# honglianghe/CDNet

Measured on AMD Instinct MI355X. Metric: tiles/sec (train fwd+bwd+Adam), 256x256, higher is better.
Workload: dtype fp32

## Files before the change

cdnet_amd/_lib.py:

```python
import ctypes as C
import os

_HERE = os.path.dirname(os.path.abspath(__file__))
LIB_PATH = os.environ.get('CDNET_LIB_PATH') or os.path.join(_HERE, 'libcdnet_hip.so')

_vp, _i, _sz, _f = C.c_void_p, C.c_int, C.c_size_t, C.c_float

class WgradReduceDesc(C.Structure):
    _fields_ = [('slab', C.c_void_p), ('dw', C.c_void_p)] + [(n, C.c_int) for n in (
        'ksplit', 'npar', 'ci_blocks', 'co_blocks', 'taps', 'CI', 'CO', 'Csrc_real', 'Cin_real', 'src_coff', 'Cout', 'mode', 'block0', 'blocks')]


SIGNATURES = {
    'cdnet_abi_version': (_i, []),
    'cdnet_abi_sizeof': (_sz, [C.c_char_p]),
    'cdnet_last_error': (C.c_char_p, []),
    'cdnet_build_info': (C.c_char_p, []),
    'cdnet_spin': (_i, [_i, _vp]),
    'cdnet_box_copy': (_i, [_vp, _vp, _sz, _vp]),
    'cdnet_box_mfma': (_i, [_vp, _vp, _vp, _i, _i, _i, _vp]),
    'cdnet_ddm_codes': (_i, [_vp, _i, _i, _i, _i, _vp, _i, _i, _vp, _vp, _vp]),
    'cdnet_ddm_normalize': (_i, [_vp, _vp, _i, _i, _i, _vp, _vp]),
    'cdnet_probmaps': (_i, [_vp, _vp, _i, _i, _i, _i, _vp, _vp, _vp]),
    'cdnet_tta_boost_argmax': (_i, [_vp, _vp, _vp, _vp, _i, _i, _vp, _i, _i, _vp, _vp, _vp, _vp, _vp, _vp]),
    'cdnet_fuse_sum': (_i, [_vp, _i, _i, _i, _i, _i, _i, _vp, _i, _i, _vp]),
    'cdnet_upsample_bilinear_backward': (_i, [_vp, _i, _i, _i, _i, _i, _i, _i, _i, _vp, _vp]),
    'cdnet_s2d_to_nhwc': (_i, [_vp, _i, _i, _i, _i, _vp, _vp]),
    'cdnet_fuse_sum_f32': (_i, [_vp, _i, _i, _i, _i, _i, _i, _vp, _i, _i, _vp]),
    'cdnet_upsample_bilinear_backward_f32': (_i, [_vp, _i, _i, _i, _i, _i, _i, _i, _i, _vp, _vp]),
    'cdnet_s2d_to_nhwc_f32': (_i, [_vp, _i, _i, _i, _i, _vp, _vp]),
    'cdnet_bn_backward_stats': (_i, [_vp, _vp, _vp, _vp, _vp, _sz, _vp, _vp]),
    'cdnet_bn_backward_apply': (_i, [_vp, _vp, _vp, _vp]),
    'cdnet_bn_backward_finalize': (_i, [_vp, _vp, _vp, _vp, _vp, _i, _vp, _vp]),
    'cdnet_conv_ws_eligible': (_i, [_vp]),
    'cdnet_grad_sum': (_i, [_vp, _i, _vp, C.c_longlong, _i, _vp, _vp]),
    'cdnet_grad_sum_f32': (_i, [_vp, _i, _vp, C.c_longlong, _i, _vp, _vp]),
    'cdnet_label_pair_histogram': (_i, [_vp, _vp, _i, _i, _i, _i, _vp, _vp, _vp, _vp, _vp, _vp]),
    'cdnet_remap_label': (_i, [_vp, _i, _i, _i, _vp, _vp, _vp, _vp]),
    'cdnet_watershed_workspace_bytes': (_sz, [_i, _i, _i]),
    'cdnet_watershed_process': (_i, [_vp, _i, _i, _i, _i, _vp, _sz, _vp, _vp, _vp, _vp]),
    'cdnet_fill_label_process': (_i, [_vp, _i, _i, _i, _i, _vp, _sz, _vp, _vp]),
    'cdnet_tile_postproc_workspace_bytes': (_sz, [_i, _i, _i, _i]),
    'cdnet_tile_postproc': (_i, [_vp, _vp, _vp, _i, _i, _i, _i, _vp, _i, _i, _i, _i, _vp, _sz] + [_vp] * 10),
    'cdnet_cc_workspace_bytes': (_sz, [_i, _i, _i]),
    'cdnet_cc_chain': (_i, [_vp, _i, _i, _i, _i, _i, _i, _vp, _sz, _vp, _vp, _vp, _vp, _vp, _vp]),
    'cdnet_mask_views_argmax': (_i, [_vp, _i, _i, _i, _vp, _i, _i, _vp, _vp, _vp]),
    'cdnet_tile_mask_postproc_workspace_bytes': (_sz, [_i, _i, _i, _i]),
    'cdnet_tile_mask_postproc': (_i, [_vp, _i, _i, _i, _i, _i, _i, _vp, _sz] + [_vp] * 8),
    'cdnet_dilate_labels': (_i, [_vp, _i, _i, _i, _i, _vp, _vp]),
    'cdnet_conv_packed_weight_elems': (_sz, [_i] * 6),
    'cdnet_pack_conv_weights': (_i, [_vp, _vp] + [_i] * 7 + [_vp]),
    'cdnet_pack_conv_weights_scaled': (_i, [_vp, _vp, _vp] + [_i] * 7 + [_vp]),
    'cdnet_pack_batch_table_bytes': (_sz, [_i]),
    'cdnet_pack_conv_weights_batch': (_i, [_vp, _i, _vp, _sz, _i, _vp]),
    'cdnet_conv_forward': (_i, [_vp, _vp]),
    'cdnet_src_materialize': (_i, [_vp, _i, _i, _i, _vp, _vp]),
    'cdnet_input_pack': (_i, [_vp, _i, _i, _i, _i, _vp, _vp]),
    'cdnet_input_pack_f32': (_i, [_vp, _i, _i, _i, _i, _vp, _vp]),
    'cdnet_bn_fold_eval': (_i, [_vp, _vp, _vp, _vp, _vp, _f, _i, _vp, _vp, _vp]),
    'cdnet_bn_finalize_train': (_i, [_vp, _i, _i, _f, _vp, _vp, _vp, _f, _f, _vp, _vp, _vp, _vp, _vp, _vp, _vp]),
    'cdnet_dam_head_forward': (_i, [_vp, _vp, _vp, _vp, _i, _i, _i, _vp, _vp, _vp, _vp]),
    'cdnet_final_conv1x1': (_i, [_vp, _vp, _vp, _i, _i, _i, _i, _vp, _vp]),
    'cdnet_bias_grad_workspace_floats': (_sz, [_i]),
    'cdnet_bias_grad': (_i, [_vp, _sz, _i, _vp, _sz, _vp, _vp]),
    'cdnet_bias_grad_f32': (_i, [_vp, _sz, _i, _vp, _sz, _vp, _vp]),
    'cdnet_final_conv1x1_backward_workspace_floats': (_sz, []),
    'cdnet_final_conv1x1_backward': (_i, [_vp, _vp, _vp, _i, _i, _i, _i, _vp, _vp, _sz, _vp, _vp, _vp]),
# ... 102 lines not shown
```

cdnet_amd/csrc/conv32.hip:

```cpp
#include <type_traits>
#include "common.h"
#include "conv_args.h"
#include "launch.h"
#include <stdlib.h>

using namespace cdnet;

typedef __attribute__((ext_vector_type(8))) __bf16 bf16x8;
typedef __attribute__((ext_vector_type(2))) __bf16 bf16x2;
typedef __attribute__((ext_vector_type(16))) float f32x16;
typedef __attribute__((ext_vector_type(2))) float f32x2;
typedef unsigned u32x4 __attribute__((ext_vector_type(4)));
typedef float f32x4 __attribute__((ext_vector_type(4)));

namespace {

__device__ __forceinline__ void split8(const float *v, u32x4 &hi, u32x4 &lo) {
#pragma unroll
    for (int k = 0; k < 4; ++k) {
        const f32x2 x = {v[2 * k], v[2 * k + 1]};
        const bf16x2 h = __builtin_convertvector(x, bf16x2);
        const unsigned hb = __builtin_bit_cast(unsigned, h);
        const f32x2 hf = {__builtin_bit_cast(float, hb << 16), __builtin_bit_cast(float, hb & 0xffff0000u)};
        const bf16x2 l = __builtin_convertvector(x - hf, bf16x2);
        hi[k] = hb;
        lo[k] = __builtin_bit_cast(unsigned, l);
    }
}

constexpr int CK = 16;
constexpr int PSTR = CK * 2 + 16;
constexpr int XF_MAX = 2048;

template <int TH, int TW, int BN, int TAPS>
struct Lds32 {
    static constexpr int NPIX = (TH + 2) * (TW + 2);
    static constexpr int A_PLANE = NPIX * PSTR;
    static constexpr int B_PLANE = TAPS * CK * BN * 2;
    static constexpr int STAGE = 2 * A_PLANE + 2 * B_PLANE;
    static constexpr int STATS_BYTES = 4 * 2 * BN * 4;
    static constexpr int MAIN = ((STAGE > STATS_BYTES ? STAGE : STATS_BYTES) + 15) / 16 * 16;
    static int bytes(int ctot) { return MAIN + 2 * ((ctot + 7) / 8 * 8) * 4; }
};


template <int MPW, int NPW, int TW>
__device__ __forceinline__ void store_tile_f32(const ConvArgs &A, const f32x16 (&acc)[MPW][NPW], int n, int y0, int x0, int mblock0, int nblock0,
                                               int half, int l31, int cout0, int pa_, int pb_) {
    const int Ho = A.H * A.ostride, Wo = A.W * A.ostride;
    float *out = reinterpret_cast<float *>(A.out);
    const float *eres = reinterpret_cast<const float *>(A.eres);
    const bool full = y0 + 16 <= A.H && x0 + TW <= A.W && cout0 + (nblock0 + NPW) * 32 <= A.Cout && A.ostride == 1 && TW == 16 &&
                      !(A.debug & 16);
    if (full) {
        const int cs = A.out_cstride, ce = A.Cout;
        float *tb = out + (((size_t)n * A.H + y0) * A.W + x0) * cs + A.out_coff;
        const float *te = eres ? eres + (((size_t)n * A.H + y0) * A.W + x0) * ce : nullptr;
#pragma unroll
        for (int ni = 0; ni < NPW; ++ni) {
            const int co = cout0 + (nblock0 + ni) * 32 + l31;
            const float osc = A.oscale ? A.oscale[co] : 1.f;
            const float osh = fmaf(A.bias ? A.bias[co] : 0.f, osc, A.oshift ? A.oshift[co] : 0.f);
            const float esc = (eres && A.eres_scale) ? A.eres_scale[co] : 1.f;
            const float esh = (eres && A.eres_shift) ? A.eres_shift[co] : 0.f;
            float *ob = tb + co;
#pragma unroll
            for (int mi = 0; mi < MPW; ++mi) {
                const int rowb = ((mblock0 + mi) * 2) * A.W + 4 * half;
                float ev[16];
                if (eres) {
#pragma unroll
                    for (int r = 0; r < 16; ++r) {
                        const int p = (r & 3) + 8 * (r >> 2);
                        ev[r] = te[(rowb + (p / 16) * A.W + (p % 16)) * ce + co];
                    }
                }
#pragma unroll
                for (int r = 0; r < 16; ++r) {
                    const int p = (r & 3) + 8 * (r >> 2);
                    const int off = (rowb + (p / 16) * A.W + (p % 16)) * cs;
                    float v = fmaf(acc[mi][ni][r], osc, osh);
                    if (A.orelu) v = fmaxf(v, 0.f);
                    if (eres) {
                        v = fmaf(ev[r], esc, esh) + v;
                        if (A.eres_relu) v = fmaxf(v, 0.f);
                    }
// ... 12 lines not shown
        const float esc = (A.eres && A.eres_scale && cok) ? A.eres_scale[co] : 1.f;
        const float esh = (A.eres && A.eres_shift && cok) ? A.eres_shift[co] : 0.f;
#pragma unroll
        for (int mi = 0; mi < MPW; ++mi) {
            float ev[16];
            if (A.eres) {
#pragma unroll
                for (int r = 0; r < 16; ++r) {
                    const int m = (mblock0 + mi) * 32 + (r & 3) + 8 * (r >> 2) + 4 * half;
                    int y = y0 + m / TW, x = x0 + m % TW;
                    y = y < A.H ? y : A.H - 1; x = x < A.W ? x : A.W - 1;
                    ev[r] = eres[(((size_t)n * A.H + y) * A.W + x) * A.Cout + (cok ? co : 0)];
                }
            }
#pragma unroll
            for (int r = 0; r < 16; ++r) {
                const int m = (mblock0 + mi) * 32 + (r & 3) + 8 * (r >> 2) + 4 * half;
                const int y = y0 + m / TW, x = x0 + m % TW;
                float v = fmaf(acc[mi][ni][r], osc, osh);
                if (A.orelu) v = fmaxf(v, 0.f);
                if (A.eres) {
                    v = fmaf(ev[r], esc, esh) + v;
                    if (A.eres_relu) v = fmaxf(v, 0.f);
                }
                if (cok && y < A.H && x < A.W) {
                    const size_t opix = ((size_t)n * Ho + (y * A.ostride + pa_)) * Wo + (x * A.ostride + pb_);
                    out[opix * A.out_cstride + A.out_coff + co] = v;
                }
            }
        }
    }
}

template <int TH, int TW, int BN, int WM, int WN, int TAPS>
__global__ __launch_bounds__(256, 2) void conv_f32_kernel(ConvArgs A) {
    using L = Lds32<TH, TW, BN, TAPS>;
    constexpr int HW_ = TW + 2, NPIX = L::NPIX;
    constexpr int MT = TH * TW / 32, NT = BN / 32;
    constexpr int MPW = MT / WM, NPW = NT / WN;
    constexpr int VPP = CK / 8;
    constexpr int NA = (NPIX * VPP + 255) / 256;
    constexpr int NBV = 2 * L::B_PLANE / 16;
    constexpr int NB = (NBV + 255) / 256;
    static_assert(MT % WM == 0 && NT % WN == 0 && WM * WN == 4, "wave tiling");

    extern __shared__ __attribute__((aligned(16))) unsigned char smem[];
    unsigned char *lds_a = smem;
    unsigned char *lds_b = smem + 2 * L::A_PLANE;
    float (*s_stats)[2][BN] = reinterpret_cast<float (*)[2][BN]>(smem);
    float *s_xf = reinterpret_cast<float *>(smem + L::MAIN);

    const int tid = threadIdx.x, lane = tid & 63, wave = tid >> 6;
    const int wm = wave / WN, wn = wave % WN;
    const int half = lane >> 5, l31 = lane & 31;
    const int c0n = A.src[0].C, ctot = c0n + (A.nsrc > 1 ? A.src[1].C : 0);
    const int xfs = (ctot + 7) / 8 * 8;
    for (int c = tid; c < ctot; c += 256) {
        const ConvSrc &S = c < c0n ? A.src[0] : A.src[1];
        const int cc = c < c0n ? c : c - c0n;
        s_xf[c] = S.scale ? S.scale[cc] : 1.f;
        s_xf[xfs + c] = S.shift ? S.shift[cc] : 0.f;
    }

    const int tiles_x = (A.W + TW - 1) / TW, tiles_y = (A.H + TH - 1) / TH;
    const int tiles_img = tiles_x * tiles_y;
    int tile, cout_tile;
    {
        const int NC = (int)gridDim.y, lin = (int)blockIdx.y * (int)gridDim.x + (int)blockIdx.x;
        const int T = (int)gridDim.x * NC, q = T >> 3, rem = T & 7;
        const int xcd = lin & 7, idx = lin >> 3;
        const int seq = xcd < rem ? xcd * (q + 1) + idx : rem * (q + 1) + (xcd - rem) * q + idx;
        tile = seq / NC;
        cout_tile = seq - tile * NC;
    }
    const int z = tile / tiles_img, rt = tile - z * tiles_img;
    const int n = z / A.npar, par = z - n * A.npar;
    const int ty_ = rt / tiles_x;
    const int y0 = ty_ * TH, x0 = (rt - ty_ * tiles_x) * TW;

    int eoff[2][NA];
    const int slot = tid % VPP;
#pragma unroll
    for (int si = 0; si < 2; ++si) {
        if (si >= A.nsrc) break;
        const ConvSrc &s = A.src[si];
        const int rs = s.row_stride ? s.row_stride : s.Ws * s.C;
#pragma unroll
        for (int i = 0; i < NA; ++i) {
            const int v = tid + i * 256;
            const int pix = v / VPP;
            const int hy = pix / HW_, hx = pix - hy * HW_;
            const int y = y0 - 1 + hy, x = x0 - 1 + hx;
            const int ys = y - s.off_y, xs = x - s.off_x;
            const bool ok = v < NPIX * VPP && (unsigned)y < (unsigned)A.H && (unsigned)x < (unsigned)A.W && (unsigned)ys < (unsigned)s.Hs &&
                            (unsigned)xs < (unsigned)s.Ws;
            eoff[si][i] = ok ? ys * rs + xs * s.C + slot * 8 : -1;
        }
    }
    auto chunk_src = [&](int c, int &si, int &cc0) {
        const int n0 = A.src[0].C / CK;
        if (c < n0) { si = 0; cc0 = c * CK; } else { si = 1; cc0 = (c - n0) * CK; }
    };
    const unsigned short *wbase = A.w + ((size_t)(par * gridDim.y + cout_tile) * A.nchunk) * (size_t)(L::B_PLANE);

    f32x4 pa[NA][2];
    u32x4 pb[NB];
    auto issue = [&](int chunk) {
        int si, cc0;
        chunk_src(chunk, si, cc0);
        const ConvSrc &s = A.src[si];
        const size_t rs = s.row_stride ? (size_t)s.row_stride : (size_t)s.Ws * s.C;
        const float *base = reinterpret_cast<const float *>(s.x) + (size_t)n * s.Hs * rs + cc0;
#pragma unroll
        for (int i = 0; i < NA; ++i) {
            const int e = si ? eoff[1][i] : eoff[0][i];
            const f32x4 *p = reinterpret_cast<const f32x4 *>(base + (e >= 0 ? e : 0));
            pa[i][0] = p[0];
            pa[i][1] = p[1];
        }
        const u32x4 *wsrc = reinterpret_cast<const u32x4 *>(wbase + (size_t)chunk * L::B_PLANE);
#pragma unroll
        for (int i = 0; i < NB; ++i) {
            const int v = tid + i * 256;
            if (v < NBV) pb[i] = wsrc[v];
        }
    };
    auto commit = [&](int chunk) {
        int si, cc0;
        chunk_src(chunk, si, cc0);
        const ConvSrc &s = A.src[si];
        const bool on = s.scale != nullptr, relu = s.relu != 0;
        const float *xf = s_xf + (si ? c0n : 0) + cc0 + slot * 8;
        float sc[8], sh[8];
        if (on) {
#pragma unroll
            for (int j = 0; j < 8; ++j) { sc[j] = xf[j]; sh[j] = xf[xfs + j]; }
        }
        f32x4 rr[NA][2];
        if (s.res) {
            const size_t rs = s.row_stride ? (size_t)s.row_stride : (size_t)s.Ws * s.C;
            const float *rbase = reinterpret_cast<const float *>(s.res) + (size_t)n * s.Hs * rs + cc0;
#pragma unroll
            for (int i = 0; i < NA; ++i) {
                const int e = si ? eoff[1][i] : eoff[0][i];
                const f32x4 *p = reinterpret_cast<const f32x4 *>(rbase + (e >= 0 ? e : 0));
                rr[i][0] = p[0];
                rr[i][1] = p[1];
            }
        }
        unsigned char *dst0 = lds_a + (tid / VPP) * PSTR + slot * 16;
#pragma unroll
        for (int i = 0; i < NA; ++i) {
            if (tid + i * 256 >= NPIX * VPP) continue;
            const int e = si ? eoff[1][i] : eoff[0][i];
            u32x4 hi = {0u, 0u, 0u, 0u}, lo = {0u, 0u, 0u, 0u};
            if (e >= 0) {
                float v[8] = {pa[i][0][0], pa[i][0][1], pa[i][0][2], pa[i][0][3], pa[i][1][0], pa[i][1][1], pa[i][1][2], pa[i][1][3]};
                if (on) {
#pragma unroll
                    for (int j = 0; j < 8; ++j) v[j] = fmaf(v[j], sc[j], sh[j]);
                }
                if (s.res) {
                    const float r[8] = {rr[i][0][0], rr[i][0][1], rr[i][0][2], rr[i][0][3], rr[i][1][0], rr[i][1][1], rr[i][1][2], rr[i][1][3]};
#pragma unroll
                    for (int j = 0; j < 8; ++j) v[j] += r[j];
                }
                if (relu) {
#pragma unroll
                    for (int j = 0; j < 8; ++j) v[j] = fmaxf(v[j], 0.f);
                }
                split8(v, hi, lo);
            }
            unsigned char *d = dst0 + i * (256 / VPP) * PSTR;
            *reinterpret_cast<u32x4 *>(d) = hi;
            *reinterpret_cast<u32x4 *>(d + L::A_PLANE) = lo;
        }
        u32x4 *bdst = reinterpret_cast<u32x4 *>(lds_b);
#pragma unroll
        for (int i = 0; i < NB; ++i) {
            const int v = tid + i * 256;
            if (v < NBV) bdst[v] = pb[i];
        }
    };

    int abase[MPW];
#pragma unroll
    for (int mi = 0; mi < MPW; ++mi) {
        const int m = (wm * MPW + mi) * 32 + l31;
        abase[mi] = ((m / TW) * HW_ + m % TW) * PSTR + half * 16;
    }
    const int bbase = half * BN * 16 + (wn * NPW * 32 + l31) * 16;
    int toff[TAPS];
#pragma unroll
    for (int t = 0; t < TAPS; ++t) {
        int r, c;
        if (TAPS == 9) { r = t / 3; c = t % 3; }
        else if (TAPS == 4) {
            const int a = par >> 1, b = par & 1, ty = t >> 1, tx = t & 1;
            r = a == 0 ? (ty == 0 ? 1 : 0) : (ty == 0 ? 2 : 1);
            c = b == 0 ? (tx == 0 ? 1 : 0) : (tx == 0 ? 2 : 1);
        } else { r = 1; c = 1; }
        toff[t] = (r * HW_ + c) * PSTR;
    }
    f32x16 acc[MPW][NPW];
#pragma unroll
    for (int mi = 0; mi < MPW; ++mi)
#pragma unroll
        for (int ni = 0; ni < NPW; ++ni)
#pragma unroll
            for (int r = 0; r < 16; ++r) acc[mi][ni][r] = 0.f;

    issue(0);
    for (int chunk = 0; chunk < A.nchunk; ++chunk) {
        __syncthreads();
        commit(chunk);
        __syncthreads();
        if (chunk + 1 < A.nchunk) issue(chunk + 1);
#pragma unroll
        for (int t = 0; t < TAPS; ++t) {
            bf16x8 ah[MPW], al[MPW], bh[NPW], bl[NPW];
#pragma unroll
            for (int mi = 0; mi < MPW; ++mi) {
                ah[mi] = *reinterpret_cast<const bf16x8 *>(lds_a + abase[mi] + toff[t]);
                al[mi] = *reinterpret_cast<const bf16x8 *>(lds_a + L::A_PLANE + abase[mi] + toff[t]);
            }
#pragma unroll
            for (int ni = 0; ni < NPW; ++ni) {
                bh[ni] = *reinterpret_cast<const bf16x8 *>(lds_b + bbase + t * 2 * BN * 16 + ni * 512);
                bl[ni] = *reinterpret_cast<const bf16x8 *>(lds_b + L::B_PLANE + bbase + t * 2 * BN * 16 + ni * 512);
            }
#pragma unroll
            for (int mi = 0; mi < MPW; ++mi)
#pragma unroll
                for (int ni = 0; ni < NPW; ++ni) {
                    acc[mi][ni] = __builtin_amdgcn_mfma_f32_32x32x16_bf16(al[mi], bh[ni], acc[mi][ni], 0, 0, 0);
                    acc[mi][ni] = __builtin_amdgcn_mfma_f32_32x32x16_bf16(ah[mi], bl[ni], acc[mi][ni], 0, 0, 0);
                    acc[mi][ni] = __builtin_amdgcn_mfma_f32_32x32x16_bf16(ah[mi], bh[ni], acc[mi][ni], 0, 0, 0);
                }
        }
    }
    __syncthreads();

    const int cout0 = cout_tile * BN;
    if (A.stats) {
        float ssum[NPW], ssq[NPW];
        const bool full_tile = y0 + TH <= A.H && x0 + TW <= A.W && !(A.debug & 16);
#pragma unroll
        for (int ni = 0; ni < NPW; ++ni) {
            ssum[ni] = 0.f; ssq[ni] = 0.f;
            if (full_tile) {
#pragma unroll
                for (int mi = 0; mi < MPW; ++mi)
#pragma unroll
                    for (int r = 0; r < 16; ++r) {
                        const float v = acc[mi][ni][r];
                        ssum[ni] += v;
                        ssq[ni] = fmaf(v, v, ssq[ni]);
                    }
            } else {
#pragma unroll
            for (int mi = 0; mi < MPW; ++mi)
#pragma unroll
                for (int r = 0; r < 16; ++r) {
                    const int m = (wm * MPW + mi) * 32 + (r & 3) + 8 * (r >> 2) + 4 * half;
                    const float v = ((y0 + m / TW) < A.H && (x0 + m % TW) < A.W) ? acc[mi][ni][r] : 0.f;
                    ssum[ni] += v;
                    ssq[ni] = fmaf(v, v, ssq[ni]);
                }
            }
            ssum[ni] += __shfl_xor(ssum[ni], 32);
            ssq[ni] += __shfl_xor(ssq[ni], 32);
            if (half == 0) {
                s_stats[wave][0][(wn * NPW + ni) * 32 + l31] = ssum[ni];
                s_stats[wave][1][(wn * NPW + ni) * 32 + l31] = ssq[ni];
            }
        }
        __syncthreads();
        if (tid < 2 * BN) {
            const int which = tid / BN, col = tid % BN;
            const int wn_of = col / (NPW * 32);
            float v = 0.f;
#pragma unroll
            for (int k = 0; k < WM; ++k) v += s_stats[k * WN + wn_of][which][col];
            const int co = cout0 + col;
            if (co < A.Cout) A.stats[((size_t)tile * 2 + which) * A.Cout + co] = v;
        }
    }
    store_tile_f32<MPW, NPW, TW>(A, acc, n, y0, x0, wm * MPW, wn * NPW, half, l31, cout0, par >> 1, par & 1);
}

template <int TH, int TW, int BN, int WM, int WN, int TAPS>
int launch_conv32(const ConvArgs &A, hipStream_t st) {
    using L = Lds32<TH, TW, BN, TAPS>;
    int ctot = 0;
    for (int i = 0; i < A.nsrc; ++i) ctot += A.src[i].C;
    const int smem = L::bytes(ctot);
    dim3 grid(cdiv(A.W, TW) * cdiv(A.H, TH) * A.N * A.npar, cdiv(A.Cout, BN), 1);
    return launch_lds<conv_f32_kernel<TH, TW, BN, WM, WN, TAPS>>(grid, 256, L::bytes(XF_MAX), smem, st, "hipFuncSetAttribute(conv32)", "conv_f32_kernel", A);
}

template <int TAPS>
int dispatch_conv32(const ConvArgs &A, hipStream_t st) {
    if (A.tile == 16 && A.BN == 64) return launch_conv32<16, 16, 64, 4, 1, TAPS>(A, st);
    if (A.tile == 16 && A.BN == 32) return launch_conv32<16, 16, 32, 4, 1, TAPS>(A, st);
    if (A.tile == 8 && A.BN == 64) return launch_conv32<8, 8, 64, 2, 2, TAPS>(A, st);
    set_error("cdnet_conv_forward(f32): unsupported configuration tile=%d CK=%d BN=%d", A.tile, A.CK, A.BN);
    return CDNET_E_ARG;
}

template <int BN, int NCH, bool XF, bool ERES>
__global__ __launch_bounds__(256, 4) void conv1x1_f32_stream_kernel(ConvArgs A) {
    constexpr int NPW = BN / 32;
    constexpr int B_PLANE = CK * BN * 2;
    constexpr int CIN = NCH * CK;
    __shared__ __attribute__((aligned(16))) unsigned char smem[NCH * 2 * B_PLANE + 2 * CIN * 4];
    unsigned char *lds_b = smem;
    float *s_xf = reinterpret_cast<float *>(smem + NCH * 2 * B_PLANE);

    const int tid = threadIdx.x, lane = tid & 63, wave = __builtin_amdgcn_readfirstlane(tid >> 6);
    const int half = lane >> 5, l31 = lane & 31;
    const int cout_tile = blockIdx.y, cout0 = cout_tile * BN;
    const ConvSrc &S = A.src[0];
    {
        const u32x4 *wsrc = reinterpret_cast<const u32x4 *>(A.w + (size_t)cout_tile * NCH * B_PLANE);
        u32x4 *bdst = reinterpret_cast<u32x4 *>(lds_b);
        for (int v = tid; v < NCH * 2 * B_PLANE / 16; v += 256) bdst[v] = wsrc[v];
        for (int c = tid; c < CIN; c += 256) {
            s_xf[c] = S.scale ? S.scale[c] : 1.f;
            s_xf[CIN + c] = S.shift ? S.shift[c] : 0.f;
        }
    }
    __syncthreads();

    const size_t P = (size_t)A.N * A.H * A.W;
    const int nblk = (int)((P + 31) / 32), bstride = (int)gridDim.x * 4;
    int blk = (int)blockIdx.x * 4 + wave;
    if (blk >= nblk) return;
    const bool relu = S.relu != 0, orelu = A.orelu != 0, eres_relu = A.eres_relu != 0;
// ... 195 lines not shown
                    yy = yy < s.Hs ? yy : s.Hs - 1;
                    xx = xx < s.Ws ? xx : s.Ws - 1;
                    raw[q] = *reinterpret_cast<const float4 *>(sx + img + (size_t)yy * rs + (size_t)xx * s.C + c);
                }
#pragma unroll
                for (int q = 0; q < 4; ++q) {
                    const float4 t = xf(raw[q], nullptr);
                    if (q == 0) val = t;
                    else if (ok[q]) { val.x = fmaxf(val.x, t.x); val.y = fmaxf(val.y, t.y); val.z = fmaxf(val.z, t.z); val.w = fmaxf(val.w, t.w); }
                }
            }
        }
        *reinterpret_cast<float4 *>(out + pix * s.C + c) = val;
    }
}

}

namespace cdnet {

int conv_forward_f32(const ConvArgs &A, hipStream_t st) {
    CDNET_REQUIRE(A.CK == 16, "cdnet_conv_forward(f32): CK must be 16 (got %d)", A.CK);
    for (int i = 0; i < A.nsrc; ++i)
        CDNET_REQUIRE(!A.src[i].pool, "cdnet_conv_forward(f32): pooled sources must be materialised (cdnet_src_materialize)");
    CDNET_REQUIRE(!A.out_f16, "cdnet_conv_forward(f32): out_f16 must be 0");
    {
        const int rc = conv_forward_f32_ws(A, st);
        if (rc >= 0) return rc;
    }
    CDNET_REQUIRE(A.ws != 2, "cdnet_conv_forward(f32): the BatchNorm-backward statistics epilogue (ws = 2) needs the producer / consumer kernel "
                             "(ask cdnet_conv_ws_eligible first)");
    CDNET_REQUIRE(A.taps1 == 0 || A.taps1 == A.taps, "cdnet_conv_forward(f32): a one-tap second source runs on conv_ws32_kernel only (ask cdnet_conv_ws_eligible)");
    CDNET_REQUIRE(!A.pool_out, "cdnet_conv_forward(f32): the fused max-pool output rides in conv_ws32_kernel's epilogue only (ask cdnet_conv_ws_eligible)");
    if (A.taps == 9) return dispatch_conv32<9>(A, st);
    if (A.taps == 4) return dispatch_conv32<4>(A, st);
    {
        const int rc = try_conv1x1_stream(A, st);
        if (rc >= 0) return rc;
    }
    return dispatch_conv32<1>(A, st);
}

int materialize_f32(const ConvSrc &s, int N, int H, int W, void *out, hipStream_t st) {
    const size_t total = (size_t)N * H * W * (s.C / 4);
    size_t g = (total + 255) / 256;
    g = g > 8192 ? 8192 : g;
    materialize_f32_kernel<<<(int)g, 256, 0, st>>>(s, N, H, W, reinterpret_cast<float *>(out));
    return check_launch("cdnet_src_materialize(f32)");
}

}
```

cdnet_amd/csrc/conv_args.h:

```cpp
#pragma once
#include "../../include/cdnet_hip.h"

struct ConvSrc {
    const unsigned short *x;
    const unsigned short *res;
    const float *scale;
    const float *shift;
    int C, Hs, Ws, pool, relu, off_y, off_x;
    int f16, row_stride;
};

struct ConvArgs {
    ConvSrc src[2];
    int nsrc;
    const unsigned short *w;
    const float *bias;
    const float *oscale;
    const float *oshift;
    int orelu;
    unsigned short *out;
    int Cout, out_cstride, out_coff;
    float *stats;
    int N, H, W;
    int taps, npar, ostride, nchunk;
    int tile, CK, BN;
    int out_f16;
    int debug;
    int ws;
    int f32;
    const unsigned short *eres;
    const float *eres_scale, *eres_shift;
    int eres_f16, eres_relu;
    int taps1, pad_;
    unsigned short *pool_out;
    const float *dot_w, *dot_b;
    float *dot_out;
};

enum : int {
    CONV_DBG_WS16_QUAD = 16,
    CONV_DBG_ONE_TILE = 32,
    CONV_DBG_PERSIST_SMALL = 64,
    CONV_DBG_OLD_WS16 = 128,
    CONV_DBG_NO_STREAM_1X1 = 256,
    CONV_DBG_GRID_SHIFT = 8,
};
enum : int {
    WGRAD_DBG_NO_WS = 8,
    WGRAD_DBG_ALL_QUADS = 16,
};

static_assert(sizeof(ConvSrc) == sizeof(cdnet_conv_src), "ConvSrc layout");
static_assert(sizeof(ConvArgs) == sizeof(cdnet_conv_args), "ConvArgs layout");

namespace cdnet {
int conv_forward_f32(const ConvArgs &A, hipStream_t st);
int conv_forward_f32_ws(const ConvArgs &A, hipStream_t st, bool dry_run = false);
int conv_forward_ws16(const ConvArgs &A, hipStream_t st, bool dry_run = false);
int materialize_f32(const ConvSrc &s, int N, int H, int W, void *out, hipStream_t st);
}
```

cdnet_amd/engine.py:

```python
import ctypes as C
import os
import torch

from . import _lib


class ConvSrc(C.Structure):
    _fields_ = [('x', C.c_void_p), ('res', C.c_void_p), ('scale', C.c_void_p), ('shift', C.c_void_p),
                ('C', C.c_int), ('Hs', C.c_int), ('Ws', C.c_int), ('pool', C.c_int), ('relu', C.c_int),
                ('off_y', C.c_int), ('off_x', C.c_int), ('f16', C.c_int), ('row_stride', C.c_int)]


class ConvArgs(C.Structure):
    _fields_ = [('src', ConvSrc * 2), ('nsrc', C.c_int), ('w', C.c_void_p), ('bias', C.c_void_p),
                ('oscale', C.c_void_p), ('oshift', C.c_void_p), ('orelu', C.c_int), ('out', C.c_void_p),
                ('Cout', C.c_int), ('out_cstride', C.c_int), ('out_coff', C.c_int), ('stats', C.c_void_p),
                ('N', C.c_int), ('H', C.c_int), ('W', C.c_int), ('taps', C.c_int), ('npar', C.c_int),
                ('ostride', C.c_int), ('nchunk', C.c_int), ('tile', C.c_int), ('CK', C.c_int), ('BN', C.c_int),
                ('out_f16', C.c_int), ('debug', C.c_int), ('ws', C.c_int), ('f32', C.c_int),
                ('eres', C.c_void_p), ('eres_scale', C.c_void_p), ('eres_shift', C.c_void_p), ('eres_f16', C.c_int), ('eres_relu', C.c_int),
                ('taps1', C.c_int), ('pad_', C.c_int), ('pool_out', C.c_void_p),
                ('dot_w', C.c_void_p), ('dot_b', C.c_void_p), ('dot_out', C.c_void_p)]


def _dp(t):
    return None if t is None else t.data_ptr()


class Src:

    def __init__(self, x, scale=None, shift=None, relu=False, pool=False, res=None, off=(0, 0), view=None):
        assert x.dtype in (torch.bfloat16, torch.float16, torch.float32) and x.is_contiguous()
        assert res is None or res.dtype == x.dtype
        self.x, self.scale, self.shift, self.relu, self.pool, self.res, self.off = x, scale, shift, relu, pool, res, off
        if view is None:
            assert x.dim() == 4
            self.N, self.Hs, self.Ws, self.Cc = x.shape
            self.ptr_off, self.row_stride = 0, 0
        else:
            self.ptr_off, self.Hs, self.Ws, self.Cc, self.row_stride = view
            self.N = x.shape[0]

    @property
    def f16(self):
        return {torch.bfloat16: 0, torch.float16: 1, torch.float32: 2}[self.x.dtype]

    @property
    def f32(self):
        return self.x.dtype == torch.float32

    @property
    def C(self):
        return self.Cc

# ... 105 lines not shown

PACK_SPLIT = 16


def pack_weights(w, cfg, mode, Cin_pad=None, out=None, split=False, cout_scale=None):
    assert w.dtype == torch.float32 and w.is_cuda and w.is_contiguous()
    Cout, Cin, KH, KW, CK, BN, taps, npar = _pack_dims(w, cfg, mode)
    Cin_p = Cin if Cin_pad is None else Cin_pad
    if Cin_p != Cin:
        if mode == 0:
            wp = torch.zeros((Cout, Cin_p, KH, KW), dtype=torch.float32, device=w.device)
            wp[:, :Cin] = w
        else:
            raise NotImplementedError
        w, Cin = wp.contiguous(), Cin_p
    n = packed_elems(Cout, Cin // CK, taps, CK, BN, npar) * (2 if split else 1)
    if out is None or out.numel() != n:
        out = torch.empty((n,), dtype=torch.int16, device=w.device)
    if cout_scale is not None:
        assert mode == 0 and cout_scale.dtype == torch.float32 and cout_scale.numel() == Cout
        _lib.call('cdnet_pack_conv_weights_scaled', _lib.ptr(w), _lib.ptr(cout_scale), _lib.ptr(out), Cout, Cin, KH, KW, CK, BN,
                  mode | (PACK_SPLIT if split else 0), _lib.stream_ptr())
        return out
    _lib.call('cdnet_pack_conv_weights', _lib.ptr(w), _lib.ptr(out), Cout, Cin, KH, KW, CK, BN, mode | (PACK_SPLIT if split else 0),
              _lib.stream_ptr())
    return out


CONV_DEBUG = 0


def conv_forward(srcs, wpacked, Cout, cfg, taps=9, transposed=False, bias=None, oscale=None, oshift=None,
                 orelu=False, out=None, stats=None, H=None, W=None, out_dtype=torch.bfloat16, eres=None, query_ws=False, bns=None, taps1=0, pool_out=None, dot=None,
                 pad_chunks=0, debug_or=0):
    tile, CK, BN = cfg[:3]
    s0 = srcs[0]
    f32 = s0.f32
    assert all(s.f32 == f32 for s in srcs)
    if f32:
        out_dtype = torch.float32
    N = s0.N
    if H is None:
        H, W = s0.logical_hw()
        H, W = H + 0, W + 0
    ostride = 2 if transposed else 1
    npar = 4 if transposed else 1
    a = ConvArgs()
    nchunk = 0
    for i, s in enumerate(srcs):
        assert s.C % CK == 0, (s.C, CK)
        s.fill(a.src[i])
        nchunk += s.C // CK
    a.nsrc = len(srcs)
    if dot is not None:
        assert out is None and stats is None and eres is None and bns is None and pool_out is None and not f32 and not transposed
        a.dot_w, a.dot_b, a.dot_out = dot[0].data_ptr(), dot[1].data_ptr(), dot[2].data_ptr()
        assert dot[0].numel() == Cout and dot[0].dtype == torch.float32 and dot[2].dtype == torch.float32 and dot[2].numel() == N * H * W
    elif out is None:
        out = torch.empty((N, H * ostride, W * ostride, Cout), dtype=out_dtype, device=s0.x.device)
    ntiles = ((H + tile - 1) // tile) * ((W + tile - 1) // tile)
    if stats is True:
        stats = torch.empty((N * npar * ntiles, 2, Cout), dtype=torch.float32, device=s0.x.device)
    a.w, a.bias, a.oscale, a.oshift = _dp(wpacked), _dp(bias), _dp(oscale), _dp(oshift)
    a.orelu = int(orelu)
    a.out, a.Cout, a.out_cstride, a.out_coff = (None if out is None else out.data_ptr()), Cout, (Cout if out is None else out.shape[3]), 0
    a.stats = _dp(stats)
    a.N, a.H, a.W = N, H, W
    assert pad_chunks == 0 or (len(srcs) == 2 and taps == 9 and not f32 and all(s.scale is None and not s.relu and s.res is None and not s.f16 for s in srcs))
    a.taps, a.npar, a.ostride, a.nchunk = taps, npar, ostride, nchunk + pad_chunks
    a.tile, a.CK, a.BN = tile, CK, BN
    a.out_f16 = int(out is not None and out.dtype == torch.float16)
    a.ws = 0
    a.taps1 = taps1
    a.pool_out = _dp(pool_out)
    a.debug = CONV_DEBUG | debug_or
    a.f32 = int(f32)
    assert out is None or (out.dtype == torch.float32) == f32
    if eres is not None:
        assert not transposed and stats is None and not orelu and out.dtype == (torch.float32 if f32 else torch.bfloat16) and tuple(eres.x.shape) == tuple(out.shape)
        assert eres.f32 == f32
        a.eres, a.eres_scale, a.eres_shift = eres.x.data_ptr(), _dp(eres.scale), _dp(eres.shift)
        a.eres_f16, a.eres_relu = int(eres.f16), int(eres.relu)
    if bns is not None:
        raw, sc, sh, mu, inv, partial = bns
        assert eres is None and stats is None and bias is None and oscale is None and oshift is None and tuple(raw.shape) == tuple(out.shape)
        a.ws = 2
        a.eres, a.oscale, a.oshift, a.eres_scale, a.eres_shift, a.stats = raw.data_ptr(), sc.data_ptr(), sh.data_ptr(), mu.data_ptr(), inv.data_ptr(), partial.data_ptr()
    if query_ws:
        return int(_lib.load().cdnet_conv_ws_eligible(C.byref(a)))
    _lib.call('cdnet_conv_forward', C.byref(a), _lib.stream_ptr())
    return out, stats
```

cdnet_amd/trainer.py:

```python
import ctypes as C
import os

import torch

from . import _lib, engine, optim, runtime, streams
from .allreduce import BucketReducer, bucketed_allreduce
from .engine import Src
from .optim import HEAD_PARAMS, FlatState
from .synth import synthetic_batch


class GradIn(C.Structure):
    _fields_ = [('g', C.c_void_p), ('Hg', C.c_int), ('Wg', C.c_int), ('oy', C.c_int), ('ox', C.c_int),
                ('pooled', C.c_int), ('coff', C.c_int), ('cstride', C.c_int), ('pad_', C.c_int)]


class BnBwdArgs(C.Structure):
    _fields_ = [('raw', C.c_void_p), ('res', C.c_void_p), ('scale', C.c_void_p), ('shift', C.c_void_p),
                ('mean', C.c_void_p), ('invstd', C.c_void_p), ('gin', GradIn * 3), ('ngin', C.c_int),
                ('f16', C.c_int), ('relu', C.c_int), ('N', C.c_int), ('H', C.c_int), ('W', C.c_int), ('C', C.c_int)]


_WGRAD_WGS_DEEP, _WGRAD_WGS_SHALLOW = 128, 160
_WGRAD_WGS_KQ = 128
# ... 552 lines not shown
                ws = self._ws('slab', lib.cdnet_bias_grad_workspace_floats(Cout), side=True)
                _lib.call(_lib.entry('cdnet_bias_grad', g.dtype == torch.float32), _lib.ptr(g), g.numel() // Cout, Cout,
                          _lib.ptr(ws), ws.numel(), _lib.ptr(L.bias.grad), _lib.stream_ptr())

    def _input_backward(self, L, srcs, g, H, W, add):
        if not getattr(L, 'needs_input_grad', True):
            return
        N = g.N if isinstance(g, Src) else g.shape[0]
        Cout = L.Cout
        cin_total = sum(s.C for s in srcs)
        wpb, cfgb = L.backward_pack(cin_total, H, W)
        if L.kind == 'conv3s2':
            Cp = cin_total // 4
            gs2d = self.buf(('ds2d', L.name), (N, H, W, cin_total), runtime.act_dtype())
            engine.conv_forward([Src(g)], wpb, cin_total, cfgb, taps=9, out=gs2d, H=H, W=W)
            gin = self.buf(('din', L.name), (N, 2 * H, 2 * W, Cp), runtime.act_dtype())
            _lib.call(_lib.entry('cdnet_s2d_to_nhwc', gin.dtype == torch.float32), _lib.ptr(gs2d), N, H, W, Cp, _lib.ptr(gin),
                      _lib.stream_ptr())
            add(srcs[0].x, _G(gin, 2 * H, 2 * W))
            return
        if not L.transposed:
            gin = self.buf(('din', L.name), (N, H, W, cin_total), runtime.act_dtype())
            fuse = None if isinstance(g, Src) else self._stats_fusable(L, srcs, H, W, N, wpb, cfgb, cin_total)
            if fuse is not None:
                P, part = fuse
                engine.conv_forward([Src(g)], wpb, cin_total, cfgb, taps=L.taps, out=gin, H=H, W=W,
                                    bns=(srcs[0].x, P.scale, P.shift, P.save_mean, P.save_invstd, part))
                self._bn_partials[id(srcs[0].x)] = part
            else:
                engine.conv_forward([g if isinstance(g, Src) else Src(g)], wpb, cin_total, cfgb, taps=L.taps, out=gin, H=H, W=W)
        else:
            gin = self.buf(('din', L.name), (N, H, W, cin_total), runtime.act_dtype())
            views = [Src(g, view=(a * 2 * W * Cout, H, W, 2 * Cout, 4 * W * Cout)) for a in (0, 1)]
            engine.conv_forward(views, wpb, cin_total, cfgb, taps=(9 if L.kind == 'convT4' else 1), out=gin, H=H, W=W)
        coff = 0
        for s in srcs:
            if getattr(s, 'is_input', False):
                coff += s.C
                continue
            tgt, pool = getattr(s, 'grad_to', (s.x, int(s.pool)))
            add(tgt, _G(gin, H, W, oy=s.off[0], ox=s.off[1], pooled=pool, coff=coff, cstride=cin_total))
            coff += s.C

    def _overlap_begin(self):
        self._ar = None
        if not self._reduce_active() or os.environ.get('CDNET_ALLREDUCE_OVERLAP', '1') == '0':
            return
        f = self.flat
        base = f.G.data_ptr()
        pend = {}
        owners = [p for L in self.tape if not isinstance(L, runtime.FuseNode) for p in (L.weight, L.bias, None if L.bn is None else L.bn.weight,
                                                 None if L.bn is None else L.bn.bias) if p is not None]
        for p in owners:
            off = (p.grad.data_ptr() - base) // 4
            if 0 <= off < f.n_used:
                pend[off] = off + p.numel()
        if f.n_head:
            pend[0] = f.n_head
        self._ar = BucketReducer(f.G, f.n_used, self.bucket, pend)

    def _overlap_done(self, params):
        if self._ar is None:
            return
        if params is None:
            self._ar.done([0])
        else:
            base = self.flat.G.data_ptr()
# ... 183 lines not shown
```

include/cdnet_hip.h:

```cpp
#ifndef CDNET_HIP_H
#define CDNET_HIP_H

#include <stddef.h>
#include <stdint.h>

#ifdef __cplusplus
extern "C" {
#endif

#define CDNET_OK            0
#define CDNET_E_ARG         1
#define CDNET_E_WORKSPACE   2
#define CDNET_E_LAUNCH      3

#define CDNET_ABI_VERSION   5

int         cdnet_abi_version(void);
size_t      cdnet_abi_sizeof(const char *struct_name);
const char *cdnet_last_error(void);
const char *cdnet_build_info(void);
int         cdnet_spin(int microseconds, void *stream);
int         cdnet_box_copy(const void *src, void *dst, size_t bytes, void *stream);
int         cdnet_box_mfma(const uint32_t *seed, float *sink, unsigned long long *stamps, int workgroups, int waves_per_wg, int iters, void *stream);

// ... 46 lines not shown
    int Hs, Ws;
    int pool;
    int relu;
    int off_y, off_x;
    int f16;
    int row_stride;
} cdnet_conv_src;

typedef struct cdnet_conv_args {
    cdnet_conv_src src[2];
    int nsrc;
    const uint16_t *w;
    const float *bias;
    const float *oscale;
    const float *oshift;
    int orelu;
    uint16_t *out;
    int Cout, out_cstride, out_coff;
    float *stats;
    int N, H, W;
    int taps;
    int npar;
    int ostride;
    int nchunk;
    int tile, CK, BN;
    int out_f16;
    int debug;
    int ws;
    int f32;
    const uint16_t *eres;
    const float *eres_scale, *eres_shift;
    int eres_f16, eres_relu;
    int taps1;
    int pad_;
    uint16_t *pool_out;
    const float *dot_w;
    const float *dot_b;
    float *dot_out;
} cdnet_conv_args;

size_t cdnet_conv_packed_weight_elems(int Cout, int nchunk, int taps, int CK, int BN, int npar);
#define CDNET_PACK_SPLIT 16
int cdnet_pack_conv_weights(const float *w, void *packed, int Cout, int Cin, int KH, int KW, int CK, int BN, int mode,
                            void *stream);
int cdnet_pack_conv_weights_scaled(const float *w, const float *cout_scale, void *packed, int Cout, int Cin, int KH, int KW, int CK,
                                   int BN, int mode, void *stream);
typedef struct cdnet_pack_job {
    const float *w;
    void *packed;
    int Cout, Cin, KH, KW, CK, BN, mode, pad_;
} cdnet_pack_job;
size_t cdnet_pack_batch_table_bytes(int n_jobs);
int cdnet_pack_conv_weights_batch(const cdnet_pack_job *jobs, int n_jobs, void *table, size_t table_bytes, int upload,
                                  void *stream);
int cdnet_conv_forward(const cdnet_conv_args *args, void *stream);

int cdnet_input_pack(const float *x, int N, int C, int H, int W, void *out_bf16_nhwc16, void *stream);
int cdnet_input_pack_f32(const float *x, int N, int C, int H, int W, float *out_f32_nhwc16, void *stream);
int cdnet_bn_fold_eval(const float *gamma, const float *beta, const float *running_mean, const float *running_var,
                       const float *conv_bias, float eps, int C, float *scale, float *shift, void *stream);
int cdnet_bn_finalize_train(const float *stats, int T, int C, float count, const float *gamma, const float *beta,
                            const float *conv_bias, float eps, float momentum, float *running_mean,
                            float *running_var, float *scale, float *shift, float *save_mean, float *save_invstd,
                            void *stream);

typedef struct cdnet_head_feat {
    const uint16_t *raw;
    const uint16_t *res;
    const float *scale;
    const float *shift;
    int relu;
    int f16;
} cdnet_head_feat;

#define CDNET_HEAD_WEIGHT_FLOATS 855
int cdnet_dam_head_forward(const cdnet_head_feat *f1, const cdnet_head_feat *f2, const cdnet_head_feat *f3,
                           const float *head_weights, int N, int H, int W, float *mask, float *point,
                           float *direction, void *stream);
int cdnet_final_conv1x1(const cdnet_head_feat *f, const float *w, const float *b, int K, int N, int H, int W,
                        float *out, void *stream);
size_t cdnet_bias_grad_workspace_floats(int C);
int cdnet_bias_grad(const uint16_t *grad_out, size_t npix, int C, float *workspace, size_t workspace_floats, float *db, void *stream);
int cdnet_bias_grad_f32(const float *grad_out, size_t npix, int C, float *workspace, size_t workspace_floats, float *db, void *stream);
size_t cdnet_final_conv1x1_backward_workspace_floats(void);
int cdnet_final_conv1x1_backward(const cdnet_head_feat *f, const float *w, const float *dlogits, int K, int N, int H, int W,
                                 uint16_t *df, float *workspace, size_t workspace_floats, float *dw, float *db, void *stream);

int cdnet_conv_ws_eligible(const cdnet_conv_args *args);
// ... 183 lines not shown
```

Measured before the change: 1068.

## Skip structurally zero taps in fp32 transposed-conv input-gradient launches

For the nine-tap fp32 launch that computes the input gradient of a 2x transposed convolution, only four of the nine taps are nonzero for each parity source and channel chunk. A per-chunk tap mask now skips loading those weight vectors and runs only the four live taps in the MFMA loop. The change also adds a subpixel store path for four-tap stride-2 outputs and interleaves the parity index in the tile order when the output is narrow, aiming for better write locality. It adds a new kernel specialization, and the ConvArgs padding field is reused as convt_ct.

```diff
diff --git a/cdnet_amd/_lib.py b/cdnet_amd/_lib.py
--- a/cdnet_amd/_lib.py
+++ b/cdnet_amd/_lib.py
@@ -33,6 +33,7 @@
     'cdnet_bn_backward_apply': (_i, [_vp, _vp, _vp, _vp]),
     'cdnet_bn_backward_finalize': (_i, [_vp, _vp, _vp, _vp, _vp, _i, _vp, _vp]),
     'cdnet_conv_ws_eligible': (_i, [_vp]),
+    'cdnet_convt_tap_mask': (C.c_uint, [_i, _i]),
     'cdnet_grad_sum': (_i, [_vp, _i, _vp, C.c_longlong, _i, _vp, _vp]),
     'cdnet_grad_sum_f32': (_i, [_vp, _i, _vp, C.c_longlong, _i, _vp, _vp]),
     'cdnet_label_pair_histogram': (_i, [_vp, _vp, _i, _i, _i, _i, _vp, _vp, _vp, _vp, _vp, _vp]),
diff --git a/cdnet_amd/csrc/conv32.hip b/cdnet_amd/csrc/conv32.hip
--- a/cdnet_amd/csrc/conv32.hip
+++ b/cdnet_amd/csrc/conv32.hip
@@ -44,14 +44,39 @@
 };
 
 
-template <int MPW, int NPW, int TW>
+template <int MPW, int NPW, int TW, bool SUBPIX>
 __device__ __forceinline__ void store_tile_f32(const ConvArgs &A, const f32x16 (&acc)[MPW][NPW], int n, int y0, int x0, int mblock0, int nblock0,
                                                int half, int l31, int cout0, int pa_, int pb_) {
     const int Ho = A.H * A.ostride, Wo = A.W * A.ostride;
     float *out = reinterpret_cast<float *>(A.out);
     const float *eres = reinterpret_cast<const float *>(A.eres);
-    const bool full = y0 + 16 <= A.H && x0 + TW <= A.W && cout0 + (nblock0 + NPW) * 32 <= A.Cout && A.ostride == 1 && TW == 16 &&
-                      !(A.debug & 16);
+    const bool full_sp = y0 + 16 <= A.H && x0 + TW <= A.W && TW == 16 && !(A.debug & 16);
+    const bool full = full_sp && cout0 + (nblock0 + NPW) * 32 <= A.Cout && A.ostride == 1;
+    if (SUBPIX && full_sp && A.ostride == 2 && !eres && (long long)Wo * A.out_cstride < (1LL << 31) / 32) {
+        const int cs = A.out_cstride;
+        float *tb = out + (((size_t)n * Ho + 2 * y0 + pa_) * Wo + 2 * x0 + pb_) * cs + A.out_coff;
+#pragma unroll
+        for (int ni = 0; ni < NPW; ++ni) {
+            const int co = cout0 + (nblock0 + ni) * 32 + l31;
+            if (co >= A.Cout) continue;
+            const float osc = A.oscale ? A.oscale[co] : 1.f;
+            const float osh = fmaf(A.bias ? A.bias[co] : 0.f, osc, A.oshift ? A.oshift[co] : 0.f);
+            float *ob = tb + co;
+#pragma unroll
+            for (int mi = 0; mi < MPW; ++mi) {
+                const int rowb = ((mblock0 + mi) * 4) * Wo + 8 * half;
+#pragma unroll
+                for (int r = 0; r < 16; ++r) {
+                    const int p = (r & 3) + 8 * (r >> 2);
+                    const int off = (rowb + 2 * (p / 16) * Wo + 2 * (p % 16)) * cs;
+                    float v = fmaf(acc[mi][ni][r], osc, osh);
+                    if (A.orelu) v = fmaxf(v, 0.f);
+                    ob[off] = v;
+                }
+            }
+        }
+        return;
+    }
     if (full) {
         const int cs = A.out_cstride, ce = A.Cout;
         float *tb = out + (((size_t)n * A.H + y0) * A.W + x0) * cs + A.out_coff;
@@ -130,8 +155,9 @@
     }
 }
 
-template <int TH, int TW, int BN, int WM, int WN, int TAPS>
+template <int TH, int TW, int BN, int WM, int WN, int TAPS, bool CT4 = false>
 __global__ __launch_bounds__(256, 2) void conv_f32_kernel(ConvArgs A) {
+    static_assert(!CT4 || TAPS == 9, "the tap mask belongs to nine-tap launches");
     using L = Lds32<TH, TW, BN, TAPS>;
     constexpr int HW_ = TW + 2, NPIX = L::NPIX;
     constexpr int MT = TH * TW / 32, NT = BN / 32;
@@ -171,8 +197,19 @@
         tile = seq / NC;
         cout_tile = seq - tile * NC;
     }
-    const int z = tile / tiles_img, rt = tile - z * tiles_img;
-    const int n = z / A.npar, par = z - n * A.npar;
+    int n, par, rt;
+    if (A.npar == 4 && A.out_cstride < 32 && !(A.debug & CONV_DBG_CONVT_PAR_APART)) {
+        par = tile & 3;
+        const int u = tile >> 2;
+        n = u / tiles_img;
+        rt = u - n * tiles_img;
+        tile = (n * 4 + par) * tiles_img + rt;
+    } else {
+        const int z = tile / tiles_img;
+        rt = tile - z * tiles_img;
+        n = z / A.npar;
+        par = z - n * A.npar;
+    }
     const int ty_ = rt / tiles_x;
     const int y0 = ty_ * TH, x0 = (rt - ty_ * tiles_x) * TW;
 
@@ -201,6 +238,14 @@
     };
     const unsigned short *wbase = A.w + ((size_t)(par * gridDim.y + cout_tile) * A.nchunk) * (size_t)(L::B_PLANE);
 
+    constexpr int TSTEP = 256 / (2 * BN);
+    static_assert(256 % (2 * BN) == 0, "a thread's weight vectors are whole taps apart");
+    const int tslot0 = tid / (2 * BN);
+    auto chunk_mask = [&](int c) -> unsigned {
+        int si, cc0;
+        chunk_src(c, si, cc0);
+        return convt_tap_mask(si, cc0 >= A.convt_ct ? 1 : 0);
+    };
     f32x4 pa[NA][2];
     u32x4 pb[NB];
     auto issue = [&](int chunk) {
@@ -217,10 +262,11 @@
             pa[i][1] = p[1];
         }
         const u32x4 *wsrc = reinterpret_cast<const u32x4 *>(wbase + (size_t)chunk * L::B_PLANE);
+        const unsigned m = CT4 ? chunk_mask(chunk) : 0u, m2 = m | (m << TAPS);
 #pragma unroll
         for (int i = 0; i < NB; ++i) {
             const int v = tid + i * 256;
-            if (v < NBV) pb[i] = wsrc[v];
+            if (v < NBV && (!CT4 || ((m2 >> (tslot0 + i * TSTEP)) & 1u))) pb[i] = wsrc[v];
         }
     };
     auto commit = [&](int chunk) {
@@ -274,10 +320,11 @@
             *reinterpret_cast<u32x4 *>(d + L::A_PLANE) = lo;
         }
         u32x4 *bdst = reinterpret_cast<u32x4 *>(lds_b);
+        const unsigned m = CT4 ? chunk_mask(chunk) : 0u, m2 = m | (m << TAPS);
 #pragma unroll
         for (int i = 0; i < NB; ++i) {
             const int v = tid + i * 256;
-            if (v < NBV) bdst[v] = pb[i];
+            if (v < NBV && (!CT4 || ((m2 >> (tslot0 + i * TSTEP)) & 1u))) bdst[v] = pb[i];
         }
     };
 
@@ -314,13 +361,16 @@
         commit(chunk);
         __syncthreads();
         if (chunk + 1 < A.nchunk) issue(chunk + 1);
-#pragma unroll
-        for (int t = 0; t < TAPS; ++t) {
+        const int t0 = CT4 ? __builtin_ctz(chunk_mask(chunk) | 0x100u) : 0;
+#pragma unroll
+        for (int tt = 0; tt < (CT4 ? 4 : TAPS); ++tt) {
+            const int t = CT4 ? t0 + (tt >> 1) * 3 + (tt & 1) : tt;
+            const int to = CT4 ? ((t / 3) * HW_ + t % 3) * PSTR : toff[tt];
             bf16x8 ah[MPW], al[MPW], bh[NPW], bl[NPW];
 #pragma unroll
             for (int mi = 0; mi < MPW; ++mi) {
-                ah[mi] = *reinterpret_cast<const bf16x8 *>(lds_a + abase[mi] + toff[t]);
-                al[mi] = *reinterpret_cast<const bf16x8 *>(lds_a + L::A_PLANE + abase[mi] + toff[t]);
+                ah[mi] = *reinterpret_cast<const bf16x8 *>(lds_a + abase[mi] + to);
+                al[mi] = *reinterpret_cast<const bf16x8 *>(lds_a + L::A_PLANE + abase[mi] + to);
             }
 #pragma unroll
             for (int ni = 0; ni < NPW; ++ni) {
@@ -384,24 +434,24 @@
             if (co < A.Cout) A.stats[((size_t)tile * 2 + which) * A.Cout + co] = v;
         }
     }
-    store_tile_f32<MPW, NPW, TW>(A, acc, n, y0, x0, wm * MPW, wn * NPW, half, l31, cout0, par >> 1, par & 1);
-}
-
-template <int TH, int TW, int BN, int WM, int WN, int TAPS>
+    store_tile_f32<MPW, NPW, TW, TAPS == 4>(A, acc, n, y0, x0, wm * MPW, wn * NPW, half, l31, cout0, par >> 1, par & 1);
+}
+
+template <int TH, int TW, int BN, int WM, int WN, int TAPS, bool CT4 = false>
 int launch_conv32(const ConvArgs &A, hipStream_t st) {
     using L = Lds32<TH, TW, BN, TAPS>;
     int ctot = 0;
     for (int i = 0; i < A.nsrc; ++i) ctot += A.src[i].C;
     const int smem = L::bytes(ctot);
     dim3 grid(cdiv(A.W, TW) * cdiv(A.H, TH) * A.N * A.npar, cdiv(A.Cout, BN), 1);
-    return launch_lds<conv_f32_kernel<TH, TW, BN, WM, WN, TAPS>>(grid, 256, L::bytes(XF_MAX), smem, st, "hipFuncSetAttribute(conv32)", "conv_f32_kernel", A);
-}
-
-template <int TAPS>
+    return launch_lds<conv_f32_kernel<TH, TW, BN, WM, WN, TAPS, CT4>>(grid, 256, L::bytes(XF_MAX), smem, st, "hipFuncSetAttribute(conv32)", "conv_f32_kernel", A);
+}
+
+template <int TAPS, bool CT4 = false>
 int dispatch_conv32(const ConvArgs &A, hipStream_t st) {
-    if (A.tile == 16 && A.BN == 64) return launch_conv32<16, 16, 64, 4, 1, TAPS>(A, st);
-    if (A.tile == 16 && A.BN == 32) return launch_conv32<16, 16, 32, 4, 1, TAPS>(A, st);
-    if (A.tile == 8 && A.BN == 64) return launch_conv32<8, 8, 64, 2, 2, TAPS>(A, st);
+    if (A.tile == 16 && A.BN == 64) return launch_conv32<16, 16, 64, 4, 1, TAPS, CT4>(A, st);
+    if (A.tile == 16 && A.BN == 32) return launch_conv32<16, 16, 32, 4, 1, TAPS, CT4>(A, st);
+    if (A.tile == 8 && A.BN == 64) return launch_conv32<8, 8, 64, 2, 2, TAPS, CT4>(A, st);
     set_error("cdnet_conv_forward(f32): unsupported configuration tile=%d CK=%d BN=%d", A.tile, A.CK, A.BN);
     return CDNET_E_ARG;
 }
@@ -663,6 +713,11 @@
                              "(ask cdnet_conv_ws_eligible first)");
     CDNET_REQUIRE(A.taps1 == 0 || A.taps1 == A.taps, "cdnet_conv_forward(f32): a one-tap second source runs on conv_ws32_kernel only (ask cdnet_conv_ws_eligible)");
     CDNET_REQUIRE(!A.pool_out, "cdnet_conv_forward(f32): the fused max-pool output rides in conv_ws32_kernel's epilogue only (ask cdnet_conv_ws_eligible)");
+    if (A.convt_ct) {
+        CDNET_REQUIRE(A.convt_ct > 0 && A.taps == 9 && A.nsrc == 2 && A.src[0].C == 2 * A.convt_ct && A.src[1].C == 2 * A.convt_ct,
+                      "cdnet_conv_forward(f32): convt_ct = %d wants a nine-tap launch over two row-parity sources of 2 * convt_ct channels", A.convt_ct);
+        if (A.convt_ct % CK == 0 && !(A.debug & CONV_DBG_CONVT_ALL_TAPS)) return dispatch_conv32<9, true>(A, st);
+    }
     if (A.taps == 9) return dispatch_conv32<9>(A, st);
     if (A.taps == 4) return dispatch_conv32<4>(A, st);
     {
@@ -681,3 +736,5 @@
 }
 
 }
+
+extern "C" unsigned cdnet_convt_tap_mask(int a, int b) { return convt_tap_mask(a, b); }
diff --git a/cdnet_amd/csrc/conv_args.h b/cdnet_amd/csrc/conv_args.h
--- a/cdnet_amd/csrc/conv_args.h
+++ b/cdnet_amd/csrc/conv_args.h
@@ -31,7 +31,7 @@
     const unsigned short *eres;
     const float *eres_scale, *eres_shift;
     int eres_f16, eres_relu;
-    int taps1, pad_;
+    int taps1, convt_ct;
     unsigned short *pool_out;
     const float *dot_w, *dot_b;
     float *dot_out;
@@ -43,12 +43,19 @@
     CONV_DBG_PERSIST_SMALL = 64,
     CONV_DBG_OLD_WS16 = 128,
     CONV_DBG_NO_STREAM_1X1 = 256,
+    CONV_DBG_CONVT_ALL_TAPS = 512,
+    CONV_DBG_CONVT_PAR_APART = 1024,
     CONV_DBG_GRID_SHIFT = 8,
 };
 enum : int {
     WGRAD_DBG_NO_WS = 8,
     WGRAD_DBG_ALL_QUADS = 16,
 };
+
+__host__ __device__ constexpr unsigned convt_tap_mask(int a, int b) {
+    const unsigned rows = a == 0 ? 6u : (a == 1 ? 3u : 0u), cols = b == 0 ? 6u : (b == 1 ? 3u : 0u);
+    return ((rows & 1u) * cols) | (((rows >> 1) & 1u) * cols << 3) | (((rows >> 2) & 1u) * cols << 6);
+}
 
 static_assert(sizeof(ConvSrc) == sizeof(cdnet_conv_src), "ConvSrc layout");
 static_assert(sizeof(ConvArgs) == sizeof(cdnet_conv_args), "ConvArgs layout");
diff --git a/cdnet_amd/engine.py b/cdnet_amd/engine.py
--- a/cdnet_amd/engine.py
+++ b/cdnet_amd/engine.py
@@ -19,7 +19,7 @@
                 ('ostride', C.c_int), ('nchunk', C.c_int), ('tile', C.c_int), ('CK', C.c_int), ('BN', C.c_int),
                 ('out_f16', C.c_int), ('debug', C.c_int), ('ws', C.c_int), ('f32', C.c_int),
                 ('eres', C.c_void_p), ('eres_scale', C.c_void_p), ('eres_shift', C.c_void_p), ('eres_f16', C.c_int), ('eres_relu', C.c_int),
-                ('taps1', C.c_int), ('pad_', C.c_int), ('pool_out', C.c_void_p),
+                ('taps1', C.c_int), ('convt_ct', C.c_int), ('pool_out', C.c_void_p),
                 ('dot_w', C.c_void_p), ('dot_b', C.c_void_p), ('dot_out', C.c_void_p)]
 
 
@@ -191,7 +191,7 @@
 
 def conv_forward(srcs, wpacked, Cout, cfg, taps=9, transposed=False, bias=None, oscale=None, oshift=None,
                  orelu=False, out=None, stats=None, H=None, W=None, out_dtype=torch.bfloat16, eres=None, query_ws=False, bns=None, taps1=0, pool_out=None, dot=None,
-                 pad_chunks=0, debug_or=0):
+                 pad_chunks=0, debug_or=0, convt_ct=0):
     tile, CK, BN = cfg[:3]
     s0 = srcs[0]
     f32 = s0.f32
@@ -231,6 +231,7 @@
     a.out_f16 = int(out is not None and out.dtype == torch.float16)
     a.ws = 0
     a.taps1 = taps1
+    a.convt_ct = convt_ct if f32 else 0
     a.pool_out = _dp(pool_out)
     a.debug = CONV_DEBUG | debug_or
     a.f32 = int(f32)
diff --git a/cdnet_amd/trainer.py b/cdnet_amd/trainer.py
--- a/cdnet_amd/trainer.py
+++ b/cdnet_amd/trainer.py
@@ -608,7 +608,8 @@
         else:
             gin = self.buf(('din', L.name), (N, H, W, cin_total), runtime.act_dtype())
             views = [Src(g, view=(a * 2 * W * Cout, H, W, 2 * Cout, 4 * W * Cout)) for a in (0, 1)]
-            engine.conv_forward(views, wpb, cin_total, cfgb, taps=(9 if L.kind == 'convT4' else 1), out=gin, H=H, W=W)
+            engine.conv_forward(views, wpb, cin_total, cfgb, taps=(9 if L.kind == 'convT4' else 1), out=gin, H=H, W=W,
+                                convt_ct=(Cout if L.kind == 'convT4' else 0))
         coff = 0
         for s in srcs:
             if getattr(s, 'is_input', False):
diff --git a/include/cdnet_hip.h b/include/cdnet_hip.h
--- a/include/cdnet_hip.h
+++ b/include/cdnet_hip.h
@@ -102,7 +102,7 @@
     const float *eres_scale, *eres_shift;
     int eres_f16, eres_relu;
     int taps1;
-    int pad_;
+    int convt_ct;
     uint16_t *pool_out;
     const float *dot_w;
     const float *dot_b;
@@ -124,6 +124,7 @@
 int cdnet_pack_conv_weights_batch(const cdnet_pack_job *jobs, int n_jobs, void *table, size_t table_bytes, int upload,
                                   void *stream);
 int cdnet_conv_forward(const cdnet_conv_args *args, void *stream);
+unsigned cdnet_convt_tap_mask(int a, int b);
 
 int cdnet_input_pack(const float *x, int N, int C, int H, int W, void *out_bf16_nhwc16, void *stream);
 int cdnet_input_pack_f32(const float *x, int N, int C, int H, int W, float *out_f32_nhwc16, void *stream);
```

Measured after the change: 1072 (median of 6 runs). Within noise of the previous version (+0.4%).
